# phoboslab/jsmpeg

Measured on AMD Instinct MI355X. Metric: 1080p MPEG-1 decode throughput, higher is better.
Workload: dtype int32

## Files before the change

jsmpeg_amd/csrc/kernels.h:

```cpp
#ifndef JSMPEG_AMD_KERNELS_H
#define JSMPEG_AMD_KERNELS_H

#include <hip/hip_runtime.h>

#include "enqueue_plan.h"
#include "mpeg1_dev.h"
#include "select_plan.h"
#include "tensor_plan.h"
#include "vlc_lut.h"

#define JM_SCAN_PIECE_BYTES 16384u
#ifndef JM_SCAN_MAX_SUBS
#define JM_SCAN_MAX_SUBS 7u
#endif
static_assert(JM_SCAN_MAX_SUBS >= 1 && JM_SCAN_MAX_SUBS * 5462u < 65536u, "k_scan: a chunk's start-code count must fit 16 bits");
static_assert(JM_SCAN_MAX_SUBS * 4u * 256u * 4u <= 60u * 1024u, "k_scan: the match table must fit the LDS of one workgroup");
static inline size_t jm_scan_state_bytes(uint64_t n_bytes) {
	return sizeof(uint64_t) * (size_t)(2 + 2 * ((n_bytes + JM_SCAN_PIECE_BYTES - 1) / JM_SCAN_PIECE_BYTES + 1));
}

struct JmScanBufs {
	const uint8_t *es;
	uint32_t n_bytes;
	uint64_t *state;
	uint32_t *sc_pos;
	uint8_t *sc_code;
	uint32_t *pic_sc;
	uint32_t *slice_sc;
	uint32_t *sc_owner;
	uint32_t *counters;
	uint32_t sc_cap, pic_cap;
	uint32_t pos_bias;
};
#define JM_N_COUNTERS 8
hipError_t jm_launch_scan(const JmScanBufs &b, hipStream_t st);

hipError_t jm_launch_to_host(void *host_a, const void *dev_a, size_t bytes_a, void *host_b, const void *dev_b, size_t bytes_b, hipStream_t st);
hipError_t jm_launch_place(const uint8_t *src, uint8_t *dst, const uint32_t *src_begin, const uint32_t *dst_begin, const uint32_t *len,
                           uint32_t n_streams, uint32_t max_len, hipStream_t st);

struct JmIndexBufs {
	const uint8_t *es;
	const uint32_t *sc_pos;
	const uint8_t *sc_code;
	uint32_t *sc_owner;
	const uint32_t *pic_sc;
	const uint32_t *counters;
	JmStream *streams;
	JmPic *pics;
	uint32_t *counters_rw;
	uint32_t n_streams, sc_cap, pic_cap;
	int width, height;
};
hipError_t jm_launch_index(const JmIndexBufs &b, hipStream_t st);

struct JmSelectBufs {
	JmPic *pics;
	const JmStream *streams;
	uint32_t *sc_owner;
	uint32_t *counters;
	JmSelectLayout layout;
	uint32_t *frame_pic;
	int32_t *before_last;
	uint32_t n_streams, pic_cap;
};
hipError_t jm_launch_select(const JmSelectBufs &b, hipStream_t st);

#define JM_ORDER_BINS 1024u
struct JmOrderBufs {
	const uint32_t *slice_sc;
	const uint32_t *sc_pos;
	const uint32_t *sc_owner;
	const uint32_t *counters;
	uint32_t sc_cap, es_bytes;
	uint32_t *hist;
	uint32_t *order;
};
hipError_t jm_launch_order(const JmOrderBufs &b, hipStream_t st);

#define JM_PARSE_CU_KEYS 4096u
struct JmParseBufs {
	const uint8_t *es;
	const uint32_t *sc_pos;
	const uint8_t *sc_code;
	const uint32_t *sc_owner;
	const JmPic *pics;
	const JmStream *streams;
	const JmVlcLuts *luts;
	JmMbRec *mb;
	uint16_t *tokens;
	uint32_t n_sc;
	const uint32_t *slice_sc;
	uint32_t n_lanes;
	uint32_t *ticket;
	uint32_t *cu_order;
	uint32_t n_batches;
	int mb_size;
	uint32_t *covered;
	uint8_t epoch;
	uint32_t lanes_per_wave;
	int cold_threshold;
	uint32_t bytes_per_mb_x16;
	uint32_t t_cold;
	uint32_t split_service;
	uint32_t prio_batches;
	uint32_t long_slices;
	uint32_t head_batches[2], head_lanes[2], head_first[3];
	int debug_flags;
	uint32_t *dbg;
	const JmDevPlan *plan;
};
hipError_t jm_launch_parse(const JmParseBufs &b, hipStream_t st);
hipError_t jm_launch_parse_planned(const JmParseBufs &b, hipStream_t st);
JmParseOverrides jm_parse_overrides();

struct alignas(64) JmReconDesc {
	const uint16_t *tok;
	const JmMbRec *mb;
	uint8_t *dst;
	const uint8_t *fwd;
	const uint8_t *stale;
	const uint8_t *qm;
	uint32_t done_pic, wait_fwd, wait_stale, pad_;
};
static_assert(sizeof(JmReconDesc) == 64, "JmReconDesc: one 64-byte line, two scalar loads");

struct JmReconBufs {
	JmGeom g;
	const JmReconDesc *desc;
	uint32_t n_level_pics;
	const JmVlcLuts *luts;
	uint8_t epoch;
	int zero_uncovered;
	uint32_t need;
	uint32_t *done;
	uint32_t patience;
	uint32_t *status;
	uint32_t no_forward;
};
#define JM_RECON_STATUS_WORDS 16
#define JM_DONE_STRIDE 32
hipError_t jm_launch_recon(const JmReconBufs &b, hipStream_t st);
uint32_t jm_recon_tiles_per_picture(const JmGeom &g);

struct JmPlanDescBufs {
	JmReconDesc *desc;
	const uint16_t *tokens;
	const JmMbRec *mb;
	uint8_t *pool;
	uint64_t frame_bytes;
};
hipError_t jm_launch_plan(const JmPlanArgs &a, const JmPlanDescBufs &d, hipStream_t st);

hipError_t jm_launch_hash(const uint8_t *pool, uint64_t frame_bytes, uint32_t hashed_bytes, uint32_t n_frames,
                          uint64_t *out, hipStream_t st, const uint32_t *slots = nullptr);

struct JmRgbaBufs {
	const uint8_t *frames;
	uint32_t first_frame, n_frames;
	uint64_t frame_stride;
	uint32_t luma_bytes, chroma_bytes;
	int32_t coded_width, coded_height, width, height;
	uint8_t *rgba;
	uint64_t rgba_stride;
};
hipError_t jm_launch_rgba(const JmRgbaBufs &b, hipStream_t st);
hipError_t jm_launch_rgba_gl(const JmRgbaBufs &b, hipStream_t st);

struct JmTensorBufs {
	const uint8_t *pool;
	uint64_t frame_bytes;
	uint32_t luma_bytes, chroma_bytes;
	int32_t coded_width;
	const uint32_t *slots;
	uint32_t count;
	void *out;
};
hipError_t jm_launch_tensor(const JmTensorBufs &b, const JmTensorPlan &p, hipStream_t st);

struct JmTsRec {
	uint32_t w0;
	uint32_t w1;
	int32_t total;
	uint32_t pts_lo;
};
struct JmTsCand { uint32_t packet, flags, pos, bytes; };
struct JmTsWrite { uint32_t pts_lo, pts_hi, begin, length; };
struct JmTsBufs {
	const uint8_t *ts;
	const uint64_t *ts_begin, *ts_len;
	const uint32_t *pkt_first;
	uint32_t n_streams, stream_id;
	JmTsRec *rec;
	uint32_t *es_off;
	JmTsCand *cand;
	JmTsWrite *writes;
	uint32_t *n_writes, *es_total, *es_given, *status;
	uint8_t *es;
	const uint32_t *es_begin;
};
hipError_t jm_launch_ts_parse_walk(const JmTsBufs &b, uint32_t max_packets, hipStream_t st);
hipError_t jm_launch_ts_gather(const JmTsBufs &b, uint32_t max_packets, hipStream_t st);

#endif
```

jsmpeg_amd/csrc/kernels.hip:

```cpp
#include "kernels.h"

#include <stdlib.h>

#if defined(__HIP_DEVICE_COMPILE__) && !defined(__gfx950__)
#error "jsmpeg_amd kernels are gfx950 (MI355X) only: build with --offload-arch=gfx950"
#endif

#include "index_tables.h"
#include "recon_block.h"
#include "slice_parse.h"

#define JM_WG 256

#define JM_SCAN_AGG 1ull
#define JM_SCAN_INC 2ull

static __device__ __forceinline__ uint64_t scan_state_load(const uint64_t *p) {
	return __hip_atomic_load(p, __ATOMIC_RELAXED, __HIP_MEMORY_SCOPE_AGENT);
}
static __device__ __forceinline__ void scan_state_store(uint64_t *p, uint64_t v) {
	__hip_atomic_store(p, v, __ATOMIC_RELAXED, __HIP_MEMORY_SCOPE_AGENT);
}
static __device__ __forceinline__ uint64_t wave_sum64(uint64_t x) {
#pragma unroll
	for (int d = 32; d >= 1; d >>= 1) {
		const uint32_t lo = __shfl_xor((uint32_t)x, d, 64), hi = __shfl_xor((uint32_t)(x >> 32), d, 64);
		x += ((uint64_t)hi << 32) | lo;
	}
	return x;
}
static __device__ void scan_look_back(const uint64_t *state, uint32_t chunk, int lane, uint64_t &sum0, uint64_t &sum1) {
	sum0 = sum1 = 0;
	bool open0 = true, open1 = true;
	for (int64_t first = (int64_t)chunk - 1; first >= 0 && (open0 || open1); first -= 64) {
		const int64_t p = first - lane;
		uint64_t v0, v1;
		for (;;) {
			v0 = p >= 0 ? scan_state_load(state + 2 + 2 * p) : (JM_SCAN_INC << 62);
			v1 = p >= 0 ? scan_state_load(state + 3 + 2 * p) : (JM_SCAN_INC << 62);
			if (!__any((v0 >> 62) == 0 || (v1 >> 62) == 0)) break;
			__builtin_amdgcn_s_sleep(2);
		}
		if (open0) {
			const uint64_t inc = __ballot((v0 >> 62) == JM_SCAN_INC), val = v0 & ((1ull << 62) - 1);
			const int nearest = inc ? __ffsll((unsigned long long)inc) - 1 : 63;
			sum0 += wave_sum64(lane <= nearest ? val : 0);
			open0 = inc == 0;
		}
		if (open1) {
			const uint64_t inc = __ballot((v1 >> 62) == JM_SCAN_INC), val = v1 & ((1ull << 62) - 1);
			const int nearest = inc ? __ffsll((unsigned long long)inc) - 1 : 63;
			sum1 += wave_sum64(lane <= nearest ? val : 0);
			open1 = inc == 0;
		}
	}
}

__global__ __launch_bounds__(JM_WG) void k_scan(JmScanBufs b, uint32_t n_chunks, uint32_t subs) {
	__shared__ uint32_t s_chunk;
	__shared__ uint32_t wave_tot[2][JM_WG / 64][2];
	__shared__ uint32_t s_base[3];
	__shared__ uint32_t kept[JM_SCAN_MAX_SUBS][4][JM_WG];
	const int lane = threadIdx.x & 63, wave = threadIdx.x >> 6;
	if (threadIdx.x == 0) s_chunk = atomicAdd(reinterpret_cast<uint32_t *>(b.state), 1u);
	__syncthreads();
	const uint32_t chunk = s_chunk;
	if (chunk >= n_chunks) return;
	const uint32_t off0 = chunk * subs * JM_SCAN_PIECE_BYTES + threadIdx.x * 64u;

	uint32_t run0 = 0, run1 = 0;
	for (uint32_t sub = 0; sub < subs; sub++) {
		const uint32_t off = off0 + sub * JM_SCAN_PIECE_BYTES;
		uint32_t w[17];
#pragma unroll
		for (int k = 0; k < 4; k++) {
			uint4 v = make_uint4(~0u, ~0u, ~0u, ~0u);
			if (off + 16u * k < b.n_bytes) v = *reinterpret_cast<const uint4 *>(b.es + off + 16u * k);
			w[4 * k] = v.x; w[4 * k + 1] = v.y; w[4 * k + 2] = v.z; w[4 * k + 3] = v.w;
		}
		w[16] = off + 64u < b.n_bytes ? *reinterpret_cast<const uint32_t *>(b.es + off + 64u) : ~0u;
		uint32_t nz[17];
#pragma unroll
		for (int k = 0; k < 17; k++) nz[k] = ((w[k] & 0x7f7f7f7fu) + 0x7f7f7f7fu) | w[k];
		uint32_t hit[2] = { 0, 0 }, pic[2] = { 0, 0 }, slc[2] = { 0, 0 };
#pragma unroll
		for (int k = 0; k < 16; k++) {
			uint32_t cand = ~(nz[k] | __builtin_amdgcn_alignbit(nz[k + 1], nz[k], 8)) & 0x80808080u;
			while (cand) {
				const uint32_t j = (uint32_t)(__ffs(cand) - 1) >> 3;
				cand &= cand - 1;
				const uint32_t q = jm_alignbyte(w[k + 1], w[k], j);
				if ((q & 0x00ff0000u) == 0x00010000u && off + 4u * k + j + 3u < b.n_bytes) {
					const uint32_t code = q >> 24, bit = 1u << ((4 * k + j) & 31);
					hit[k >> 3] |= bit;
					if (code == JM_CODE_PICTURE) pic[k >> 3] |= bit;
					if (code - 1u < 0xAFu) slc[k >> 3] |= bit;
				}
			}
		}
		const uint32_t mine0 = (uint32_t)(__popc(hit[0]) + __popc(hit[1])) | ((uint32_t)(__popc(pic[0]) + __popc(pic[1])) << 16);
		const uint32_t mine1 = (uint32_t)(__popc(slc[0]) + __popc(slc[1]));
		uint32_t v0 = mine0, v1 = mine1;
#pragma unroll
		for (int d = 1; d < 64; d <<= 1) {
			const uint32_t t0 = __shfl_up(v0, d, 64), t1 = __shfl_up(v1, d, 64);
			if (lane >= d) { v0 += t0; v1 += t1; }
		}
		if (lane == 63) { wave_tot[sub & 1][wave][0] = v0; wave_tot[sub & 1][wave][1] = v1; }
		__syncthreads();
		uint32_t tot0 = 0, tot1 = 0;
#pragma unroll
		for (int i = 0; i < JM_WG / 64; i++) {
			const uint32_t t0 = wave_tot[sub & 1][i][0], t1 = wave_tot[sub & 1][i][1];
			if (i < wave) { v0 += t0; v1 += t1; }
			tot0 += t0; tot1 += t1;
		}
		kept[sub][0][threadIdx.x] = hit[0]; kept[sub][1][threadIdx.x] = hit[1];
		kept[sub][2][threadIdx.x] = run0 + v0 - mine0; kept[sub][3][threadIdx.x] = run1 + v1 - mine1;
		run0 += tot0; run1 += tot1;
	}
	if (wave == 0) {
		const uint64_t own0 = ((uint64_t)(run0 & 0xffffu) << 31) | (run0 >> 16), own1 = run1;
		if (lane == 0 && chunk > 0) {
			scan_state_store(b.state + 2 + 2 * (uint64_t)chunk, (JM_SCAN_AGG << 62) | own0);
			scan_state_store(b.state + 3 + 2 * (uint64_t)chunk, (JM_SCAN_AGG << 62) | own1);
		}
		uint64_t before0, before1;
		scan_look_back(b.state, chunk, lane, before0, before1);
		if (lane == 0) {
			scan_state_store(b.state + 2 + 2 * (uint64_t)chunk, (JM_SCAN_INC << 62) | (before0 + own0));
			scan_state_store(b.state + 3 + 2 * (uint64_t)chunk, (JM_SCAN_INC << 62) | (before1 + own1));
			s_base[0] = (uint32_t)(before0 >> 31); s_base[1] = (uint32_t)(before0 & 0x7fffffffu); s_base[2] = (uint32_t)before1;
			if (chunk == n_chunks - 1) {
				b.counters[0] = (uint32_t)((before0 + own0) >> 31);
				b.counters[1] = (uint32_t)((before0 + own0) & 0x7fffffffu);
				b.counters[4] = (uint32_t)(before1 + own1);
			}
		}
	}
	__syncthreads();
	for (uint32_t sub = 0; sub < subs; sub++) {
		const uint32_t h0 = kept[sub][0][threadIdx.x], h1 = kept[sub][1][threadIdx.x];
		if ((h0 | h1) == 0) continue;
		const uint32_t e0 = kept[sub][2][threadIdx.x], e1 = kept[sub][3][threadIdx.x];
		uint32_t sc_i = s_base[0] + (e0 & 0xffffu), pic_i = s_base[1] + (e0 >> 16), slc_i = s_base[2] + e1;
		const uint32_t off = off0 + sub * JM_SCAN_PIECE_BYTES;
#pragma unroll
		for (int h = 0; h < 2; h++) {
			uint32_t m = h ? h1 : h0;
			while (m) {
				const uint32_t pos = off + 32u * h + (uint32_t)(__ffs(m) - 1);
				m &= m - 1;
				const uint32_t code = b.es[pos + 3];
				if (sc_i < b.sc_cap) {
					b.sc_pos[sc_i] = pos + b.pos_bias;
					b.sc_code[sc_i] = (uint8_t)code;
					if (b.sc_owner) b.sc_owner[sc_i] = JM_NONE;
					if (code - 1u < 0xAFu) { if (b.slice_sc) b.slice_sc[slc_i] = sc_i; slc_i++; }
				} else b.counters[2] = 1;
				if (code == JM_CODE_PICTURE) {
					if (pic_i < b.pic_cap) b.pic_sc[pic_i] = sc_i; else b.counters[2] = 1;
					pic_i++;
				}
				sc_i++;
			}
		}
	}
}

hipError_t jm_launch_scan(const JmScanBufs &b, hipStream_t st) {
	uint32_t subs = b.n_bytes / (JM_SCAN_PIECE_BYTES * 2048u);
	subs = subs < 1 ? 1 : (subs > JM_SCAN_MAX_SUBS ? JM_SCAN_MAX_SUBS : subs);
	const uint32_t chunk_bytes = subs * JM_SCAN_PIECE_BYTES;
	uint32_t n_chunks = (b.n_bytes + chunk_bytes - 1) / chunk_bytes;
	if (n_chunks == 0) n_chunks = 1;
	hipError_t e = hipMemsetAsync(b.state, 0, sizeof(uint64_t) * (2 + 2 * (size_t)n_chunks), st);
	if (e != hipSuccess) return e;
	hipLaunchKernelGGL(k_scan, dim3(n_chunks), dim3(JM_WG), 0, st, b, n_chunks, subs);
	return hipGetLastError();
}

#define JM_PLACE_CHUNK 65536u
__global__ __launch_bounds__(JM_WG) void k_place(const uint8_t *src, uint8_t *dst, const uint32_t *src_begin, const uint32_t *dst_begin,
                                                const uint32_t *len) {
	const uint32_t s = blockIdx.y, n = len[s], c0 = blockIdx.x * JM_PLACE_CHUNK;
	if (c0 >= n) return;
	const uint32_t c1 = min(n, c0 + JM_PLACE_CHUNK);
	const uint8_t *ps = src + src_begin[s];
	uint8_t *pd = dst + dst_begin[s];
	if ((((uintptr_t)ps ^ (uintptr_t)pd) & 15u) == 0) {
		uint32_t a = c0;
		const uint32_t mis = (uint32_t)((16u - ((uintptr_t)(pd + c0) & 15u)) & 15u);
		const uint32_t head = min(mis, c1 - c0);
		if (threadIdx.x < head) pd[c0 + threadIdx.x] = ps[c0 + threadIdx.x];
		a += head;
		const uint32_t n16 = (c1 - a) >> 4;
		for (uint32_t i = threadIdx.x; i < n16; i += JM_WG)
			reinterpret_cast<uint4 *>(pd + a)[i] = reinterpret_cast<const uint4 *>(ps + a)[i];
		a += n16 << 4;
		if (a + threadIdx.x < c1) pd[a + threadIdx.x] = ps[a + threadIdx.x];
	} else {
		uint32_t a = c0;
		const uint32_t mis = (uint32_t)((16u - ((uintptr_t)(pd + c0) & 15u)) & 15u);
		const uint32_t head = min(mis, c1 - c0);
		if (threadIdx.x < head) pd[c0 + threadIdx.x] = ps[c0 + threadIdx.x];
		a += head;
		const uint32_t n16 = (c1 - a) >> 4;
		const uint32_t r = (uint32_t)((uintptr_t)(ps + a) & 15u), sh = r & 3u;
		const uint4 *base = reinterpret_cast<const uint4 *>(ps + a - r);
		for (uint32_t i = threadIdx.x; i < n16; i += JM_WG) {
			const uint4 A = base[i], B = base[i + 1];
			uint4 o;
			switch (r >> 2) {
			case 0: o = make_uint4(jm_alignbyte(A.y, A.x, sh), jm_alignbyte(A.z, A.y, sh), jm_alignbyte(A.w, A.z, sh), jm_alignbyte(B.x, A.w, sh)); break;
			case 1: o = make_uint4(jm_alignbyte(A.z, A.y, sh), jm_alignbyte(A.w, A.z, sh), jm_alignbyte(B.x, A.w, sh), jm_alignbyte(B.y, B.x, sh)); break;
			case 2: o = make_uint4(jm_alignbyte(A.w, A.z, sh), jm_alignbyte(B.x, A.w, sh), jm_alignbyte(B.y, B.x, sh), jm_alignbyte(B.z, B.y, sh)); break;
			default: o = make_uint4(jm_alignbyte(B.x, A.w, sh), jm_alignbyte(B.y, B.x, sh), jm_alignbyte(B.z, B.y, sh), jm_alignbyte(B.w, B.z, sh)); break;
			}
			reinterpret_cast<uint4 *>(pd + a)[i] = o;
		}
		a += n16 << 4;
		if (a + threadIdx.x < c1) pd[a + threadIdx.x] = ps[a + threadIdx.x];
	}
}

__global__ __launch_bounds__(JM_WG) void k_to_host(uint4 *dst_a, const uint4 *src_a, uint32_t n_a, uint4 *dst_b, const uint4 *src_b, uint32_t n_b) {
	const uint32_t i = blockIdx.x * JM_WG + threadIdx.x;
	if (i < n_a) dst_a[i] = src_a[i];
	else if (i - n_a < n_b) dst_b[i - n_a] = src_b[i - n_a];
}

hipError_t jm_launch_to_host(void *host_a, const void *dev_a, size_t bytes_a, void *host_b, const void *dev_b, size_t bytes_b, hipStream_t st) {
	const uint32_t n_a = (uint32_t)((bytes_a + 15) / 16), n_b = (uint32_t)((bytes_b + 15) / 16);
	if (n_a + n_b == 0) return hipSuccess;
	hipLaunchKernelGGL(k_to_host, dim3((n_a + n_b + JM_WG - 1) / JM_WG), dim3(JM_WG), 0, st, (uint4 *)host_a, (const uint4 *)dev_a, n_a, (uint4 *)host_b, (const uint4 *)dev_b, n_b);
	return hipGetLastError();
}

hipError_t jm_launch_place(const uint8_t *src, uint8_t *dst, const uint32_t *src_begin, const uint32_t *dst_begin, const uint32_t *len,
                           uint32_t n_streams, uint32_t max_len, hipStream_t st) {
	if (n_streams == 0 || max_len == 0) return hipSuccess;
	hipLaunchKernelGGL(k_place, dim3((max_len + JM_PLACE_CHUNK - 1) / JM_PLACE_CHUNK, n_streams), dim3(JM_WG), 0, st, src, dst, src_begin, dst_begin, len);
	return hipGetLastError();
}

__device__ __forceinline__ int jm_wg_scan_add(int *buf, int v) {
	buf[threadIdx.x] = v;
	__syncthreads();
	for (uint32_t d = 1; d < JM_WG; d <<= 1) {
		const int t = threadIdx.x >= d ? buf[threadIdx.x - d] : 0;
		__syncthreads();
		buf[threadIdx.x] += t;
		__syncthreads();
	}
	return buf[threadIdx.x];
}
__device__ __forceinline__ int jm_wg_scan_max(int *buf, int v) {
	buf[threadIdx.x] = v;
	__syncthreads();
	for (uint32_t d = 1; d < JM_WG; d <<= 1) {
		const int t = threadIdx.x >= d ? buf[threadIdx.x - d] : INT_MIN;
		__syncthreads();
		buf[threadIdx.x] = max(buf[threadIdx.x], t);
		__syncthreads();
	}
	return buf[threadIdx.x];
}

__global__ __launch_bounds__(JM_WG) void k_index(JmIndexBufs b) {
	__shared__ JmStream st;
	__shared__ uint64_t m_bits[2];
	__shared__ int has_matrices;
	__shared__ int scan[JM_WG];
	__shared__ int carry[3];
	const uint32_t s = blockIdx.x;
	if (b.counters[2]) return;
	uint32_t n_sc = b.counters[0], n_pics = b.counters[1];
	if (n_sc > b.sc_cap) n_sc = b.sc_cap;
	if (n_pics > b.pic_cap) n_pics = b.pic_cap;
	__shared__ uint32_t bound[4];
	if (threadIdx.x == 0) st = b.streams[s];
	__syncthreads();
	if (threadIdx.x < 2) bound[threadIdx.x] = jm_lower_bound(b.sc_pos, n_sc, threadIdx.x ? jm_index_stream_hi_key(st) : st.es_begin);
	__syncthreads();
	if (threadIdx.x < 2) bound[2 + threadIdx.x] = jm_lower_bound(b.pic_sc, n_pics, bound[threadIdx.x]);
	__syncthreads();
	if (threadIdx.x == 0) {
		st.sc_lo = bound[0]; st.sc_hi = bound[1]; st.pic_lo = bound[2]; st.pic_hi = bound[3];
		uint64_t ib = JM_NO_MATRIX, nb = JM_NO_MATRIX;
		has_matrices = jm_index_stream_scalars(st, b.es, b.sc_pos, b.sc_code, b.width, b.height, &ib, &nb);
		m_bits[0] = ib; m_bits[1] = nb;
		carry[0] = 0; carry[1] = -1; carry[2] = 0;
	}
	__syncthreads();
	if (has_matrices && threadIdx.x < 64) jm_index_stream_matrix(st, b.es, (int)threadIdx.x, m_bits[0], m_bits[1]);
	__syncthreads();
	int deepest = -1;
	for (uint32_t base = st.pic_lo; base < st.pic_hi; base += JM_WG) {
		const uint32_t p = base + threadIdx.x;
		const bool in = p < st.pic_hi;
		JmPic pic;
		pic.decoded = 0; pic.type = 0;
		if (in) jm_index_picture(pic, p, s, st, b.es, b.sc_pos, b.sc_code, b.pic_sc, b.sc_owner, 0, 0);
		const bool dec = in && pic.decoded;
		const int c0 = carry[0], last0 = carry[1], anchor0 = carry[2];
		__syncthreads();
		const int count = c0 + jm_wg_scan_add(scan, dec ? 1 : 0);
		__syncthreads();
		const int last_incl = max(last0, jm_wg_scan_max(scan, dec ? (int)p : -1));
		__syncthreads();
		scan[threadIdx.x] = last_incl;
		__syncthreads();
		const int prev = threadIdx.x ? scan[threadIdx.x - 1] : last0;
		__syncthreads();
		const bool anchor = dec && (pic.type != JM_PIC_PREDICTIVE || prev < 0);
		const int at_anchor = max(anchor0, jm_wg_scan_max(scan, anchor ? count : 0));
		__syncthreads();
		if (dec) {
			pic.level = count - at_anchor;
			pic.fwd = (pic.type == JM_PIC_PREDICTIVE && prev >= 0) ? prev : -1;
			deepest = max(deepest, pic.level);
		}
		if (in) b.pics[p] = pic;
		if (threadIdx.x == JM_WG - 1) { carry[0] = count; carry[1] = last_incl; carry[2] = at_anchor; }
		__syncthreads();
	}
	deepest = jm_wg_scan_max(scan, deepest);
	if (threadIdx.x == JM_WG - 1) {
		if (deepest >= 0) atomicMax(&b.counters_rw[3], (uint32_t)(deepest + 1));
		b.streams[s] = st;
	}
}

hipError_t jm_launch_index(const JmIndexBufs &b, hipStream_t st) {
	if (b.n_streams) hipLaunchKernelGGL(k_index, dim3(b.n_streams), dim3(JM_WG), 0, st, b);
	return hipGetLastError();
}

__global__ __launch_bounds__(JM_WG) void k_select(JmSelectBufs b) {
	__shared__ int scan[JM_WG];
	__shared__ int byrank[JM_WG];
	__shared__ int carry[5];
	const uint32_t s = blockIdx.x;
	if (b.counters[2]) return;
	const uint32_t lo = b.streams[s].pic_lo, hi = min(b.streams[s].pic_hi, b.pic_cap);
	const JmSelectLayout l = b.layout;
	const uint32_t nbits = l.nbits[s], off = l.off[s];
	for (uint32_t f = threadIdx.x; f < nbits; f += JM_WG) b.frame_pic[off + f] = JM_NONE;
	if (threadIdx.x == 0) { carry[0] = 0; carry[1] = -1; carry[2] = -1; carry[3] = INT_MIN; carry[4] = INT_MIN; }
	__syncthreads();
	for (uint32_t base = lo; base < hi; base += JM_WG) {
		const uint32_t p = base + threadIdx.x;
		const bool in = p < hi;
		const bool dec = in && b.pics[p].decoded;
		const int c0 = carry[0], last1 = carry[1], last2 = carry[2];
		__syncthreads();
		const int incl = jm_wg_scan_add(scan, dec ? 1 : 0);
		const int n = scan[JM_WG - 1];
		if (dec) byrank[incl - 1] = (int)p;
		__syncthreads();
		if (in) {
			b.before_last[p] = dec ? jm_select_before_last(byrank, (uint32_t)(incl - 1), last1, last2) : -1;
			if (dec) {
				const uint32_t frame = (uint32_t)(c0 + incl - 1);
				if (frame < nbits) b.frame_pic[off + frame] = p;
				if (jm_select_bit(l, s, frame)) b.pics[p].pad_ = JM_PIC_SEL_SELECTED;
			}
		}
		__syncthreads();
		if (threadIdx.x == 0) { jm_select_carry_last(byrank, (uint32_t)n, carry[1], carry[2]); carry[0] = c0 + n; }
		__syncthreads();
	}
	int needed = 0, slices = 0, levels = 0;
	for (uint32_t c = (hi - lo + JM_WG - 1) / JM_WG; c-- > 0;) {
		const uint32_t p = lo + c * JM_WG + (JM_WG - 1 - threadIdx.x);
		const bool in = p < hi;
		JmPic pic;
		pic.decoded = 0; pic.pad_ = 0; pic.level = 0;
		if (in) pic = b.pics[p];
		const bool dec = in && pic.decoded;
		const int cs = carry[3], ca = carry[4];
		__syncthreads();
		const int ns = max(cs, jm_wg_scan_max(scan, dec && (pic.pad_ & JM_PIC_SEL_SELECTED) ? -(int)p : INT_MIN));
		__syncthreads();
		const int na_incl = max(ca, jm_wg_scan_max(scan, dec && jm_select_anchor(pic) ? -(int)p : INT_MIN));
		__syncthreads();
		scan[threadIdx.x] = na_incl;
		__syncthreads();
		const int na = threadIdx.x ? scan[threadIdx.x - 1] : ca;
		if (dec) {
			if (jm_select_needed(true, ns == INT_MIN ? JM_NONE : (uint32_t)-ns, na == INT_MIN ? JM_NONE : (uint32_t)-na)) {
				needed++; slices += (int)pic.n_slices; levels = max(levels, pic.level + 1);
			} else {
				jm_select_drop(pic, b.sc_owner);
				b.pics[p] = pic;
			}
		}
		if (threadIdx.x == JM_WG - 1) { carry[3] = ns; carry[4] = na_incl; }
		__syncthreads();
	}
	needed = jm_wg_scan_add(scan, needed);
	__syncthreads();
	slices = jm_wg_scan_add(scan, slices);
	__syncthreads();
	levels = jm_wg_scan_max(scan, levels);
	if (threadIdx.x == JM_WG - 1 && needed) {
		atomicMax(&b.counters[5], (uint32_t)levels);
		atomicAdd(&b.counters[6], (uint32_t)needed);
		atomicAdd(&b.counters[7], (uint32_t)slices);
	}
}

hipError_t jm_launch_select(const JmSelectBufs &b, hipStream_t st) {
	if (b.n_streams) hipLaunchKernelGGL(k_select, dim3(b.n_streams), dim3(JM_WG), 0, st, b);
	return hipGetLastError();
}

struct JmOrderDims { uint32_t n_slices, n_sc, shift; };
static __device__ __forceinline__ JmOrderDims order_dims(const JmOrderBufs &b) {
	JmOrderDims d;
	d.n_sc = b.counters[0] < b.sc_cap ? b.counters[0] : b.sc_cap;
	d.n_slices = b.counters[4] < b.sc_cap ? b.counters[4] : b.sc_cap;
	const uint32_t mean = b.es_bytes / (d.n_slices ? d.n_slices : 1u);
	d.shift = 0;
	while ((mean >> d.shift) >= 512u) d.shift++;
	return d;
}
static __device__ __forceinline__ uint32_t order_bin(const JmOrderBufs &b, const JmOrderDims &d, uint32_t j, uint32_t &i) {
	i = b.slice_sc[j];
	if (b.sc_owner[i] == JM_NONE) return 0;
	const uint32_t len = (i + 1 < d.n_sc ? b.sc_pos[i + 1] : b.es_bytes) - b.sc_pos[i];
	const uint32_t bin = 1u + (len >> d.shift);
	return bin < JM_ORDER_BINS ? bin : JM_ORDER_BINS - 1;
}

__global__ __launch_bounds__(JM_WG) void k_order_count(JmOrderBufs b) {
	__shared__ uint32_t lh[JM_ORDER_BINS];
	const JmOrderDims d = order_dims(b);
	if (blockIdx.x * JM_WG >= d.n_slices) return;
	for (uint32_t k = threadIdx.x; k < JM_ORDER_BINS; k += JM_WG) lh[k] = 0;
	__syncthreads();
	for (uint32_t j = blockIdx.x * JM_WG + threadIdx.x; j < d.n_slices; j += gridDim.x * JM_WG) {
		uint32_t i;
		atomicAdd(&lh[order_bin(b, d, j, i)], 1u);
	}
	__syncthreads();
	for (uint32_t k = threadIdx.x; k < JM_ORDER_BINS; k += JM_WG) if (lh[k]) atomicAdd(&b.hist[k], lh[k]);
// ... 858 lines not shown
```

Baseline: 542,400.

## Coalesce start-code scan loads per wave and transpose match masks through LDS

The start-code scan now loads each wave's 4 KiB row with lane-contiguous 16-byte accesses instead of each thread reading its own 64-byte span. The one word of lookahead past each 16-byte slot comes from the next lane by shuffle, or from the next slot or a tail load at the wave edge. The per-slot 16-bit hit, picture and slice masks are written to LDS and read back in thread-owned 64-byte order, so the prefix-sum and emit phases keep their original byte ownership. This is meant to improve global load coalescing. In exchange it adds LDS traffic, a wave barrier and a 16-bit slice-offset store that assumes counts fit in 16 bits.

Measured after the change: 542,700 (median of 2 runs). Within noise of the previous version (+0.1%).

```diff
diff --git a/jsmpeg_amd/csrc/kernels.h b/jsmpeg_amd/csrc/kernels.h
--- a/jsmpeg_amd/csrc/kernels.h
+++ b/jsmpeg_amd/csrc/kernels.h
@@ -10,11 +10,12 @@
 #include "vlc_lut.h"
 
 #define JM_SCAN_PIECE_BYTES 16384u
+#define JM_SCAN_WAVE_BYTES 4096u
 #ifndef JM_SCAN_MAX_SUBS
 #define JM_SCAN_MAX_SUBS 7u
 #endif
 static_assert(JM_SCAN_MAX_SUBS >= 1 && JM_SCAN_MAX_SUBS * 5462u < 65536u, "k_scan: a chunk's start-code count must fit 16 bits");
-static_assert(JM_SCAN_MAX_SUBS * 4u * 256u * 4u <= 60u * 1024u, "k_scan: the match table must fit the LDS of one workgroup");
+static_assert(JM_SCAN_MAX_SUBS * 14u * 256u + 4096u <= 60u * 1024u, "k_scan: the match table must fit the LDS of one workgroup");
 static inline size_t jm_scan_state_bytes(uint64_t n_bytes) {
 	return sizeof(uint64_t) * (size_t)(2 + 2 * ((n_bytes + JM_SCAN_PIECE_BYTES - 1) / JM_SCAN_PIECE_BYTES + 1));
 }
diff --git a/jsmpeg_amd/csrc/kernels.hip b/jsmpeg_amd/csrc/kernels.hip
--- a/jsmpeg_amd/csrc/kernels.hip
+++ b/jsmpeg_amd/csrc/kernels.hip
@@ -60,46 +60,72 @@
 	__shared__ uint32_t s_chunk;
 	__shared__ uint32_t wave_tot[2][JM_WG / 64][2];
 	__shared__ uint32_t s_base[3];
-	__shared__ uint32_t kept[JM_SCAN_MAX_SUBS][4][JM_WG];
+	__shared__ uint32_t kept[JM_SCAN_MAX_SUBS][JM_WG];
+	__shared__ uint16_t kept_slc[JM_SCAN_MAX_SUBS][JM_WG];
+	__shared__ __attribute__((aligned(8))) uint16_t kept_hit[JM_SCAN_MAX_SUBS][4 * JM_WG];
+	__shared__ __attribute__((aligned(8))) uint16_t turn[2][4 * JM_WG];
 	const int lane = threadIdx.x & 63, wave = threadIdx.x >> 6;
 	if (threadIdx.x == 0) s_chunk = atomicAdd(reinterpret_cast<uint32_t *>(b.state), 1u);
 	__syncthreads();
 	const uint32_t chunk = s_chunk;
 	if (chunk >= n_chunks) return;
 	const uint32_t off0 = chunk * subs * JM_SCAN_PIECE_BYTES + threadIdx.x * 64u;
+	const uint32_t row0 = chunk * subs * JM_SCAN_PIECE_BYTES + wave * JM_SCAN_WAVE_BYTES;
 
 	uint32_t run0 = 0, run1 = 0;
 	for (uint32_t sub = 0; sub < subs; sub++) {
-		const uint32_t off = off0 + sub * JM_SCAN_PIECE_BYTES;
-		uint32_t w[17];
+		const uint32_t row = row0 + sub * JM_SCAN_PIECE_BYTES;
+		uint4 v[4];
 #pragma unroll
 		for (int k = 0; k < 4; k++) {
-			uint4 v = make_uint4(~0u, ~0u, ~0u, ~0u);
-			if (off + 16u * k < b.n_bytes) v = *reinterpret_cast<const uint4 *>(b.es + off + 16u * k);
-			w[4 * k] = v.x; w[4 * k + 1] = v.y; w[4 * k + 2] = v.z; w[4 * k + 3] = v.w;
-		}
-		w[16] = off + 64u < b.n_bytes ? *reinterpret_cast<const uint32_t *>(b.es + off + 64u) : ~0u;
-		uint32_t nz[17];
-#pragma unroll
-		for (int k = 0; k < 17; k++) nz[k] = ((w[k] & 0x7f7f7f7fu) + 0x7f7f7f7fu) | w[k];
-		uint32_t hit[2] = { 0, 0 }, pic[2] = { 0, 0 }, slc[2] = { 0, 0 };
-#pragma unroll
-		for (int k = 0; k < 16; k++) {
-			uint32_t cand = ~(nz[k] | __builtin_amdgcn_alignbit(nz[k + 1], nz[k], 8)) & 0x80808080u;
-			while (cand) {
-				const uint32_t j = (uint32_t)(__ffs(cand) - 1) >> 3;
-				cand &= cand - 1;
-				const uint32_t q = jm_alignbyte(w[k + 1], w[k], j);
-				if ((q & 0x00ff0000u) == 0x00010000u && off + 4u * k + j + 3u < b.n_bytes) {
-					const uint32_t code = q >> 24, bit = 1u << ((4 * k + j) & 31);
-					hit[k >> 3] |= bit;
-					if (code == JM_CODE_PICTURE) pic[k >> 3] |= bit;
-					if (code - 1u < 0xAFu) slc[k >> 3] |= bit;
+			const uint32_t at = row + 1024u * k + 16u * lane;
+			v[k] = make_uint4(~0u, ~0u, ~0u, ~0u);
+			if (at < b.n_bytes) v[k] = *reinterpret_cast<const uint4 *>(b.es + at);
+		}
+		uint32_t tail = ~0u;
+		if (lane == 63 && row + JM_SCAN_WAVE_BYTES < b.n_bytes) tail = *reinterpret_cast<const uint32_t *>(b.es + row + JM_SCAN_WAVE_BYTES);
+		uint32_t hit[4], pic[4], slc[4];
+#pragma unroll
+		for (int k = 0; k < 4; k++) {
+			uint32_t behind = __shfl_down(v[k].x, 1, 64);
+			const uint32_t wrap = k < 3 ? (uint32_t)__builtin_amdgcn_readfirstlane((int)v[k < 3 ? k + 1 : 3].x) : tail;
+			if (lane == 63) behind = wrap;
+			const uint32_t w[5] = { v[k].x, v[k].y, v[k].z, v[k].w, behind };
+			uint32_t nz[5];
+#pragma unroll
+			for (int i = 0; i < 5; i++) nz[i] = ((w[i] & 0x7f7f7f7fu) + 0x7f7f7f7fu) | w[i];
+			const uint32_t at = row + 1024u * k + 16u * lane;
+			hit[k] = pic[k] = slc[k] = 0;
+#pragma unroll
+			for (int i = 0; i < 4; i++) {
+				uint32_t cand = ~(nz[i] | __builtin_amdgcn_alignbit(nz[i + 1], nz[i], 8)) & 0x80808080u;
+				while (cand) {
+					const uint32_t j = (uint32_t)(__ffs(cand) - 1) >> 3;
+					cand &= cand - 1;
+					const uint32_t q = jm_alignbyte(w[i + 1], w[i], j);
+					if ((q & 0x00ff0000u) == 0x00010000u && at + 4u * i + j + 3u < b.n_bytes) {
+						const uint32_t code = q >> 24, bit = 1u << (4 * i + j);
+						hit[k] |= bit;
+						if (code == JM_CODE_PICTURE) pic[k] |= bit;
+						if (code - 1u < 0xAFu) slc[k] |= bit;
+					}
 				}
 			}
 		}
-		const uint32_t mine0 = (uint32_t)(__popc(hit[0]) + __popc(hit[1])) | ((uint32_t)(__popc(pic[0]) + __popc(pic[1])) << 16);
-		const uint32_t mine1 = (uint32_t)(__popc(slc[0]) + __popc(slc[1]));
+#pragma unroll
+		for (int k = 0; k < 4; k++) {
+			const uint32_t g = (uint32_t)wave * 256u + 64u * k + lane;
+			kept_hit[sub][g] = (uint16_t)hit[k]; turn[0][g] = (uint16_t)pic[k]; turn[1][g] = (uint16_t)slc[k];
+		}
+		__builtin_amdgcn_fence(__ATOMIC_RELEASE, "wavefront");
+		__builtin_amdgcn_wave_barrier();
+		__builtin_amdgcn_fence(__ATOMIC_ACQUIRE, "wavefront");
+		uint64_t m_hit, m_pic, m_slc;
+		__builtin_memcpy(&m_hit, &kept_hit[sub][4 * threadIdx.x], 8);
+		__builtin_memcpy(&m_pic, &turn[0][4 * threadIdx.x], 8);
+		__builtin_memcpy(&m_slc, &turn[1][4 * threadIdx.x], 8);
+		const uint32_t mine0 = (uint32_t)__popcll(m_hit) | ((uint32_t)__popcll(m_pic) << 16);
+		const uint32_t mine1 = (uint32_t)__popcll(m_slc);
 		uint32_t v0 = mine0, v1 = mine1;
 #pragma unroll
 		for (int d = 1; d < 64; d <<= 1) {
@@ -115,8 +141,7 @@
 			if (i < wave) { v0 += t0; v1 += t1; }
 			tot0 += t0; tot1 += t1;
 		}
-		kept[sub][0][threadIdx.x] = hit[0]; kept[sub][1][threadIdx.x] = hit[1];
-		kept[sub][2][threadIdx.x] = run0 + v0 - mine0; kept[sub][3][threadIdx.x] = run1 + v1 - mine1;
+		kept[sub][threadIdx.x] = run0 + v0 - mine0; kept_slc[sub][threadIdx.x] = (uint16_t)(run1 + v1 - mine1);
 		run0 += tot0; run1 += tot1;
 	}
 	if (wave == 0) {
@@ -140,9 +165,11 @@
 	}
 	__syncthreads();
 	for (uint32_t sub = 0; sub < subs; sub++) {
-		const uint32_t h0 = kept[sub][0][threadIdx.x], h1 = kept[sub][1][threadIdx.x];
-		if ((h0 | h1) == 0) continue;
-		const uint32_t e0 = kept[sub][2][threadIdx.x], e1 = kept[sub][3][threadIdx.x];
+		uint64_t m_hit;
+		__builtin_memcpy(&m_hit, &kept_hit[sub][4 * threadIdx.x], 8);
+		if (m_hit == 0) continue;
+		const uint32_t h0 = (uint32_t)m_hit, h1 = (uint32_t)(m_hit >> 32);
+		const uint32_t e0 = kept[sub][threadIdx.x], e1 = kept_slc[sub][threadIdx.x];
 		uint32_t sc_i = s_base[0] + (e0 & 0xffffu), pic_i = s_base[1] + (e0 >> 16), slc_i = s_base[2] + e1;
 		const uint32_t off = off0 + sub * JM_SCAN_PIECE_BYTES;
 #pragma unroll
```
